# AutonomousVehicleLaboratory/vision_semantic_segmentation

Measured on AMD Instinct MI355X. Metric: fused frames/sec/GPU (1920x1080 + 120k pts) + max|dlog-odds| vs ref, higher is better.
Workload: dtype f16 hi+lo split, MX-FP4 correction passes, fp32 accumulate

## Files before the change

include/avl_hip.h:

```cpp
#ifndef AVL_HIP_H
#define AVL_HIP_H

#include <stdint.h>

#ifdef __cplusplus
extern "C" {
#endif

#define AVL_OK 0
#define AVL_E_ARG (-1)
#define AVL_E_HIP (-2)
#define AVL_E_UNSUPPORTED (-3)

#define AVL_F32 0
#define AVL_F64 1
#define AVL_BF16 2
#define AVL_F16 3

#define AVL_MAX_MAP_CLASSES 16

const char* avl_version(void);
int avl_last_error(char* buf, int len);


// ... 134 lines not shown
    int32_t out_h, out_w, out_c, out_ld, out_rows;
    int32_t in2_ld;
    int32_t ksize, stride, pad, dil, groups;
    int32_t relu;
    int32_t out_f32;
    int32_t w_rows;
    int32_t w_layout;
    int32_t w_split;
    int32_t mx_flags;
    const void* in_lo;
    const void* in2_lo;
    void* out_lo;
    const void* w_mx;
    const void* in_mx;
    void* out_mx;
    const void* in2_mx;
    const void* in3;
    const void* in3_mx;
    int32_t in3_c, in3_ld;
    int32_t batch;
    int32_t bias_per_image;
    int32_t in_format;
    int32_t raw_batch;
} avl_seg_op;

#define AVL_IN_U8_HWC 0
#define AVL_IN_F32_CHW 1

#define AVL_MX_IN_LO 1
#define AVL_MX_RES_LO 2
#define AVL_MX_OUT_LO 4

typedef struct avl_seg_plan avl_seg_plan;

int avl_seg_plan_create(const avl_seg_op* ops_host, int n_ops, avl_seg_plan** out_plan);
void avl_seg_plan_destroy(avl_seg_plan* plan);
int avl_seg_plan_run(avl_seg_plan* plan, void* stream);
int avl_seg_plan_capture(avl_seg_plan* plan, void* stream);
int avl_seg_plan_profile(avl_seg_plan* plan, void* stream, float* ms_host, double* flops_host, double* bytes_host);
int avl_seg_plan_num_ops(const avl_seg_plan* plan);
int avl_seg_plan_nonfinite(avl_seg_plan* plan, void* stream, unsigned long long* counts_host);

#ifdef __cplusplus
}
#endif
#endif
// ... 1 lines not shown
```

vision_semantic_segmentation_amd/csrc/seg_dwpw.hip:

```cpp
#include "seg_types.h"

namespace avl {
namespace {

constexpr int TM = 128;
constexpr int TN = 256;
constexpr int A_STAGE = TM * 128;
constexpr int W_STAGE = TN * 128;
constexpr int LDS_W = 0, LDS_A = 2 * W_STAGE, LDS_P = LDS_A + 2 * A_STAGE;
constexpr int P_STEP = 8 * 6 * 8 * 4;

struct DwPwArgs {
    const void* X;
    const void* X_lo;
    const void* Wc;
    const float* bc;
    float* LG;
    unsigned char* labels;
    int ncls;
    int tiles_x;
    const void* W;
    const float* bias;
    const uint32_t* dwp;
    const int* order;
    int mtiles, per_xcd;
    void* C;
    void* C_lo;
    int H, Wd, OW, ldx, ldc, M, N, K, dil, pad, ntiles;
    unsigned x_bytes;
    int nimg;
};

typedef int v4i __attribute__((ext_vector_type(4)));

__device__ __forceinline__ void dwpw_image(DwPwArgs& p) {
    const long long ipix = (long long)p.H * p.Wd, orows = p.M;
    p.X = image_base(static_cast<const char*>(p.X), ipix, 2LL * p.ldx);
    p.X_lo = image_base(static_cast<const char*>(p.X_lo), ipix, 2LL * p.ldx);
    p.x_bytes -= (unsigned)((long long)blockIdx.z * ipix * p.ldx * 2);
    p.C = image_base(static_cast<char*>(p.C), orows, 2LL * p.ldc);
    p.C_lo = image_base(static_cast<char*>(p.C_lo), orows, 2LL * p.ldc);
    p.LG = image_base(p.LG, orows, p.ncls);
    p.labels = image_base(p.labels, orows, 1);
}

template <typename HT, int WSUB = 1>
__global__ void __launch_bounds__(512) k_dwpw(DwPwArgs p) {
    typedef typename Half16<HT>::v8 v8;
// ... 377 lines not shown
                Vec8<HT>::store(cp + 8, hi);
                if (p.C_lo) {
#pragma unroll
                    for (int i = 0; i < 8; ++i) { lo[i] -= (float)(HT)lo[i]; hi[i] -= (float)(HT)hi[i]; }
                    HT* cl = static_cast<HT*>(p.C_lo) + (long long)m * p.ldc + nbase;
                    Vec8<HT>::store(cl, lo);
                    Vec8<HT>::store(cl + 8, hi);
                }
            }
        }
    }
}

int launch_dwpw_x(const DwPwArgs& a, hipStream_t s) {
    constexpr int lds_bytes = X_LDS_P + XP_RING * FP_STEP;
    static_assert(lds_bytes <= 160 * 1024, "k_dwpw_x LDS");
    AVL_HIP_CHECK(hipFuncSetAttribute(reinterpret_cast<const void*>(&k_dwpw_x), hipFuncAttributeMaxDynamicSharedMemorySize, 160 * 1024));
    hipLaunchKernelGGL(k_dwpw_x, dim3(8 * a.per_xcd * a.ntiles, 1, a.nimg), dim3(512), lds_bytes, s, a);
    AVL_LAUNCH_CHECK();
    return AVL_OK;
}

constexpr int S_LDS_W = 0, S_LDS_AH = 2 * W_STAGE, S_LDS_AL = S_LDS_AH + 2 * A_STAGE, S_LDS_P = S_LDS_AL + 2 * A_STAGE;
template <bool CLS>
__global__ void __launch_bounds__(512) k_dwpw_xs(DwPwArgs p) {
    constexpr int PSTEP = FP_STEP;
    typedef f16 HT;
    typedef typename Half16<HT>::v8 v8;
    extern __shared__ __attribute__((aligned(16))) char lds[];
    const int tid = threadIdx.x, lane = tid & 63;
    const int wave = __builtin_amdgcn_readfirstlane(tid >> 6);
    const int wm = wave >> 2, wn = wave & 3;
    const int nt = blockIdx.x % p.ntiles;
    const int bm = blockIdx.x / p.ntiles, slot = (bm & 7) * p.per_xcd + (bm >> 3);
    if (slot >= p.mtiles) return;
    dwpw_image(p);
    const int mt = p.order[slot];
    const int nk = p.K / 64;

    const unsigned lds0 = lds_addr(lds);
    auto dma_p = [&](int s) {
        if (tid < PSTEP / 16 && s < nk)
            glds16_saddr(reinterpret_cast<const char*>(p.dwp) + s * PSTEP, (unsigned)tid * 16u, lds0 + S_LDS_P + (s & (XP_RING - 1)) * PSTEP + wave * 1024);
    };
    for (int s = 0; s < 3; ++s) dma_p(s);
    const int chunk = tid & 7, r0 = tid >> 3;
    int vbase[2];
    unsigned vmask[2];
    const int tty = p.tiles_x > 0 ? mt / p.tiles_x : 0, ttx = p.tiles_x > 0 ? mt - tty * p.tiles_x : 0;
    const int OHt = p.M / p.OW;
#pragma unroll
    for (int q = 0; q < 2; ++q) {
        const int ml = r0 + q * 64;
        int y, x;
        bool live;
        if (p.tiles_x > 0) {
            y = tty * 8 + (ml >> 4); x = ttx * 16 + (ml & 15);
            live = (y < OHt) & (x < p.OW);
        } else {
            const int m = mt * TM + ml;
            y = m / p.OW; x = m - y * p.OW;
            live = m < p.M;
        }
        vbase[q] = (int)((((long long)(y - p.pad) * p.Wd + (x - p.pad)) * p.ldx + chunk * 8) * 2);
        unsigned mk = 0;
#pragma unroll
        for (int t = 0; t < 9; ++t) {
            const int iy = y - p.pad + (t / 3) * p.dil, ix = x - p.pad + (t % 3) * p.dil;
            mk |= (unsigned)(live & (iy >= 0) & (iy < p.H) & (ix >= 0) & (ix < p.Wd)) << t;
        }
        vmask[q] = mk;
    }
    const int tstep_x = p.dil * p.ldx * 2, tstep_y = p.dil * p.Wd * p.ldx * 2;
    const char* wbase = static_cast<const char*>(p.W) + (long long)nt * TN * p.K * 4;
    unsigned w_voff;
    {
        const int r = wave * 8 + (lane >> 3);
        const int key = ((r >> 1) & 1) | (((r >> 4) & 3) << 1);
        w_voff = (unsigned)(r * p.K * 4 + (((lane & 7) ^ key) << 4));
    }
    const int w_rows64 = 64 * p.K * 4;
    auto dma_w = [&](int h) {
#pragma unroll
        for (int i = 0; i < 4; ++i) glds16_saddr(wbase + h * 128 + i * w_rows64, w_voff, lds0 + S_LDS_W + (h & 1) * W_STAGE + i * 8192 + wave * 1024);
    };
    const int fr = lane & 15, kq = lane >> 4;
    int a_sw[2], w_sw[2];
    {
        const int a_key = fr & 7, w_key = ((fr >> 1) & 1) | (((fr >> 2) & 3) << 1);
#pragma unroll
        for (int kk = 0; kk < 2; ++kk) {
            a_sw[kk] = (wm * 64 + fr) * 128 + (((kk * 4 + kq) ^ a_key) << 4);
            w_sw[kk] = S_LDS_W + (wn * 64 + (fr >> 2) * 16 + (fr & 3)) * 128 + (((kk * 4 + kq) ^ w_key) << 4);
        }
    }
    f32x4 acc[4][4];
    {
        const int nb = nt * TN + wn * 64 + kq * 16;
#pragma unroll
        for (int nj = 0; nj < 4; ++nj) {
            const float4 b = *reinterpret_cast<const float4*>(p.bias + nb + 4 * nj);
#pragma unroll
            for (int mi = 0; mi < 4; ++mi) acc[mi][nj] = f32x4{b.x, b.y, b.z, b.w};
        }
    }

    v4i rh[9], rl[9];
    const __amdgpu_buffer_rsrc_t xrsrc = __builtin_amdgcn_make_buffer_rsrc(const_cast<void*>(p.X), 0, (int)p.x_bytes, 0x00020000);
    const __amdgpu_buffer_rsrc_t xlrsrc = __builtin_amdgcn_make_buffer_rsrc(const_cast<void*>(p.X_lo), 0, (int)p.x_bytes, 0x00020000);
    auto load_taps = [&](int s, int q) {
#pragma unroll
        for (int t = 0; t < 9; ++t) {
            const int off = (vmask[q] >> t) & 1u ? vbase[q] + (t / 3) * tstep_y + (t % 3) * tstep_x : 0x7fffff00;
            rh[t] = __builtin_amdgcn_raw_buffer_load_b128(xrsrc, off, s * 128, 0);
            rl[t] = __builtin_amdgcn_raw_buffer_load_b128(xlrsrc, off, s * 128, 0);
        }
    };

    auto produce_a = [&](int s, int q) {
        float o[8];
        const float* pf = reinterpret_cast<const float*>(lds + S_LDS_P + (s & (XP_RING - 1)) * PSTEP + chunk * (10 * 8 * 4));
        {
            const float4 b0 = *reinterpret_cast<const float4*>(pf + 9 * 8), b1 = *reinterpret_cast<const float4*>(pf + 9 * 8 + 4);
            o[0] = b0.x; o[1] = b0.y; o[2] = b0.z; o[3] = b0.w;
            o[4] = b1.x; o[5] = b1.y; o[6] = b1.z; o[7] = b1.w;
        }
        float wt[9][8];
#pragma unroll
// ... 13 lines not shown
                o[2 * j + 1] = __builtin_fmaf((float)v[1], wt[t][2 * j + 1], o[2 * j + 1]);
            }
#pragma unroll
        for (int t = 0; t < 9; ++t)
#pragma unroll
            for (int j = 0; j < 4; ++j) {
                const int u = rh[t][j];
                const h2 v = __builtin_bit_cast(h2, u);
                o[2 * j] = __builtin_fmaf((float)v[0], wt[t][2 * j], o[2 * j]);
                o[2 * j + 1] = __builtin_fmaf((float)v[1], wt[t][2 * j + 1], o[2 * j + 1]);
            }
        float ol[8];
#pragma unroll
        for (int i = 0; i < 8; ++i) {
            o[i] = fmaxf(o[i], 0.f);
            ol[i] = o[i] - (float)(HT)o[i];
        }
        const int row = r0 + q * 64;
        const int sw = (s & 1) * A_STAGE + row * 128 + ((chunk ^ (row & 7)) << 4);
        Vec8<HT>::store(reinterpret_cast<HT*>(lds + S_LDS_AH + sw), o);
        Vec8<HT>::store(reinterpret_cast<HT*>(lds + S_LDS_AL + sw), ol);
    };

    dma_w(0);
    load_taps(0, 0);
    asm volatile("s_waitcnt vmcnt(18)" ::: "memory");
    __syncthreads();
    produce_a(0, 0);
    load_taps(0, 1);
    produce_a(0, 1);
    if (nk > 1) load_taps(1, 0);

    for (int s = 0; s < nk; ++s) {
        const bool more = s + 1 < nk, more2 = s + 2 < nk;
        const int ts = (s & 1) * A_STAGE;
        auto mfma_hi = [&](int kk) {
            v8 wa[4], ah[4], al[4];
#pragma unroll
            for (int nj = 0; nj < 4; ++nj) wa[nj] = *reinterpret_cast<const v8*>(lds + (kk ? w_sw[1] : w_sw[0]) + nj * 512);
#pragma unroll
            for (int mi = 0; mi < 4; ++mi) {
                ah[mi] = *reinterpret_cast<const v8*>(lds + S_LDS_AH + ts + (kk ? a_sw[1] : a_sw[0]) + mi * 2048);
                al[mi] = *reinterpret_cast<const v8*>(lds + S_LDS_AL + ts + (kk ? a_sw[1] : a_sw[0]) + mi * 2048);
            }
#pragma unroll
            for (int mi = 0; mi < 4; ++mi)
#pragma unroll
                for (int nj = 0; nj < 4; ++nj) acc[mi][nj] = Half16<HT>::mfma(wa[nj], al[mi], acc[mi][nj]);
#pragma unroll
            for (int mi = 0; mi < 4; ++mi)
#pragma unroll
                for (int nj = 0; nj < 4; ++nj) acc[mi][nj] = Half16<HT>::mfma(wa[nj], ah[mi], acc[mi][nj]);
        };
        auto mfma_lo = [&](int kk) {
            v8 wa[4], ah[4];
#pragma unroll
            for (int nj = 0; nj < 4; ++nj) wa[nj] = *reinterpret_cast<const v8*>(lds + W_STAGE + (kk ? w_sw[1] : w_sw[0]) + nj * 512);
#pragma unroll
            for (int mi = 0; mi < 4; ++mi) ah[mi] = *reinterpret_cast<const v8*>(lds + S_LDS_AH + ts + (kk ? a_sw[1] : a_sw[0]) + mi * 2048);
#pragma unroll
            for (int mi = 0; mi < 4; ++mi)
#pragma unroll
                for (int nj = 0; nj < 4; ++nj) acc[mi][nj] = Half16<HT>::mfma(wa[nj], ah[mi], acc[mi][nj]);
        };
        asm volatile("s_waitcnt lgkmcnt(0)" ::: "memory");
        __builtin_amdgcn_s_barrier();
        dma_p(s + 3);
        dma_w(2 * s + 1);
        mfma_hi(0);
        __builtin_amdgcn_sched_barrier(0);
        if (more) { produce_a(s + 1, 0); load_taps(s + 1, 1); }
        __builtin_amdgcn_sched_barrier(0);
        mfma_hi(1);
        if (more) asm volatile("s_waitcnt vmcnt(18)" ::: "memory");
        else asm volatile("s_waitcnt vmcnt(0)" ::: "memory");
        asm volatile("s_waitcnt lgkmcnt(0)" ::: "memory");
        __builtin_amdgcn_s_barrier();
        if (more) dma_w(2 * s + 2);
        mfma_lo(0);
        __builtin_amdgcn_sched_barrier(0);
        if (more) { produce_a(s + 1, 1); if (more2) load_taps(s + 2, 0); }
        __builtin_amdgcn_sched_barrier(0);
        mfma_lo(1);
        if (more2) asm volatile("s_waitcnt vmcnt(18)" ::: "memory");
        else asm volatile("s_waitcnt vmcnt(0)" ::: "memory");
    }

    int elane = lane;
    asm volatile("" : "+v"(elane));
    const int efr = elane & 15;
    if constexpr (CLS) {
        const int ekq = elane >> 4;
        __syncthreads();
#pragma unroll
        for (int mi = 0; mi < 4; ++mi) {
            const int row = wm * 64 + mi * 16 + efr;
            float v0[8], v1[8], l0[8], l1[8];
#pragma unroll
            for (int nj = 0; nj < 2; ++nj)
#pragma unroll
                for (int r = 0; r < 4; ++r) {
                    v0[nj * 4 + r] = fmaxf(acc[mi][nj][r], 0.f);
                    v1[nj * 4 + r] = fmaxf(acc[mi][2 + nj][r], 0.f);
                }
#pragma unroll
            for (int i = 0; i < 8; ++i) { l0[i] = v0[i] - (float)(HT)v0[i]; l1[i] = v1[i] - (float)(HT)v1[i]; }
            const int base = wn * A_STAGE + row * 128;
            const int o0 = base + (((2 * ekq) ^ (row & 7)) << 4), o1 = base + (((2 * ekq + 1) ^ (row & 7)) << 4);
            Vec8<HT>::store(reinterpret_cast<HT*>(lds + o0), v0);
            Vec8<HT>::store(reinterpret_cast<HT*>(lds + o1), v1);
            Vec8<HT>::store(reinterpret_cast<HT*>(lds + 65536 + o0), l0);
            Vec8<HT>::store(reinterpret_cast<HT*>(lds + 65536 + o1), l1);
        }
        __syncthreads();
        f32x4 a2[2];
#pragma unroll
        for (int t2 = 0; t2 < 2; ++t2) {
            const float4 b = *reinterpret_cast<const float4*>(p.bc + t2 * 16 + 4 * ekq);
            a2[t2] = f32x4{b.x, b.y, b.z, b.w};
        }
        const int crow = wave * 16 + efr;
        const char* wcl = static_cast<const char*>(p.Wc) + ((long long)efr * p.N + ekq * 8) * 2;
        const long long wplane = 32LL * p.N * 2;
#pragma unroll
        for (int st = 0; st < 4; ++st)
#pragma unroll
            for (int kk = 0; kk < 2; ++kk) {
                const int off = st * A_STAGE + crow * 128 + (((kk * 4 + ekq) ^ (efr & 7)) << 4);
                const v8 yh = *reinterpret_cast<const v8*>(lds + off), yl = *reinterpret_cast<const v8*>(lds + 65536 + off);
#pragma unroll
                for (int t2 = 0; t2 < 2; ++t2) {
                    const char* wp = wcl + ((long long)t2 * 16 * p.N + st * 64 + kk * 32) * 2;
                    const v8 wh = *reinterpret_cast<const v8*>(wp), wl = *reinterpret_cast<const v8*>(wp + wplane);
                    a2[t2] = Half16<HT>::mfma(wh, yl, a2[t2]);
                    a2[t2] = Half16<HT>::mfma(wl, yh, a2[t2]);
                    a2[t2] = Half16<HT>::mfma(wh, yh, a2[t2]);
                }
            }
        int m;
        {
            const int ml = crow;
            if (p.tiles_x > 0) {
                const int y = tty * 8 + (ml >> 4), x = ttx * 16 + (ml & 15);
                m = ((y < OHt) & (x < p.OW)) ? y * p.OW + x : p.M;
            } else {
                m = mt * TM + ml;
            }
        }
        constexpr int kNone = 1 << 20;
        float best = 0.f;
        int bi = kNone;
#pragma unroll
        for (int t2 = 0; t2 < 2; ++t2)
#pragma unroll
            for (int r = 0; r < 4; ++r) {
                const int cls = t2 * 16 + 4 * ekq + r;
                const float v = a2[t2][r];
                if (cls < p.ncls) {
                    if (m < p.M) p.LG[(long long)m * p.ncls + cls] = v;
                    if (bi == kNone || v > best || (v != v && best == best)) { best = v; bi = cls; }
                }
            }
#pragma unroll
        for (int sh = 16; sh <= 32; sh <<= 1) {
            const float ov = __shfl_xor(best, sh, 64);
            const int oi = __shfl_xor(bi, sh, 64);
            const bool onan = ov != ov, bnan = best != best;
            const bool better = onan ? (!bnan || oi < bi) : (!bnan && (ov > best || (ov == best && oi < bi)));
            if (oi != kNone && (bi == kNone || better)) { best = ov; bi = oi; }
        }
        if (ekq == 0 && m < p.M) p.labels[m] = (unsigned char)bi;
        return;
    }
    const int nbase = nt * TN + wn * 64 + (elane >> 4) * 16;
    if (nbase + 16 <= p.N) {
#pragma unroll
        for (int mi = 0; mi < 4; ++mi) {
            int m = mt * TM + wm * 64 + mi * 16 + efr;
            if (p.tiles_x > 0) {
                const int y = tty * 8 + wm * 4 + mi, x = ttx * 16 + efr;
                m = ((y < OHt) & (x < p.OW)) ? y * p.OW + x : p.M;
            }
            if (m < p.M) {
                float lo[8], hi[8];
#pragma unroll
                for (int nj = 0; nj < 2; ++nj)
#pragma unroll
                    for (int r = 0; r < 4; ++r) {
                        lo[nj * 4 + r] = fmaxf(acc[mi][nj][r], 0.f);
                        hi[nj * 4 + r] = fmaxf(acc[mi][2 + nj][r], 0.f);
                    }
                HT* cp = static_cast<HT*>(p.C) + (long long)m * p.ldc + nbase;
                Vec8<HT>::store(cp, lo);
                Vec8<HT>::store(cp + 8, hi);
                if (p.C_lo) {
#pragma unroll
                    for (int i = 0; i < 8; ++i) { lo[i] -= (float)(HT)lo[i]; hi[i] -= (float)(HT)hi[i]; }
                    HT* cl = static_cast<HT*>(p.C_lo) + (long long)m * p.ldc + nbase;
                    Vec8<HT>::store(cl, lo);
                    Vec8<HT>::store(cl + 8, hi);
                }
            }
        }
    }
}

template <bool CLS>
int launch_dwpw_xs(const DwPwArgs& a, hipStream_t s) {
    constexpr int lds_bytes = S_LDS_P + XP_RING * FP_STEP;
    static_assert(lds_bytes <= 160 * 1024 && S_LDS_AH == 65536 && 4 * A_STAGE == 65536, "k_dwpw_xs LDS (the classifier epilogue keeps y hi at 0 and y lo at 64 KB, 64 KB each)");
    AVL_HIP_CHECK(hipFuncSetAttribute(reinterpret_cast<const void*>(&k_dwpw_xs<CLS>), hipFuncAttributeMaxDynamicSharedMemorySize, 160 * 1024));
    hipLaunchKernelGGL(k_dwpw_xs<CLS>, dim3(8 * a.per_xcd * a.ntiles, 1, a.nimg), dim3(512), lds_bytes, s, a);
    AVL_LAUNCH_CHECK();
    return AVL_OK;
}

template <typename HT, int WSUB>
int launch_dwpw_typed(const DwPwArgs& a, int mtiles, hipStream_t s) {
    const int lds_bytes = LDS_P + (a.K / 64) * P_STEP;
    AVL_HIP_CHECK(hipFuncSetAttribute(reinterpret_cast<const void*>(&k_dwpw<HT, WSUB>), hipFuncAttributeMaxDynamicSharedMemorySize, 160 * 1024));
    hipLaunchKernelGGL((k_dwpw<HT, WSUB>), dim3(8 * a.per_xcd * a.ntiles, 1, a.nimg), dim3(512), lds_bytes, s, a);
    AVL_LAUNCH_CHECK();
    return AVL_OK;
}

}

int validate_dwpw(const avl_seg_op& op) {
    AVL_REQUIRE(is_half(op.dtype), "fused depthwise+pointwise needs a 16-bit activation type");
    AVL_REQUIRE(op.in && op.out && op.weight && op.bias && op.in2, "dwpw has NULL buffers");
    AVL_REQUIRE(!op.w_split || op.dtype == AVL_F16, "split weights need AVL_F16 activations");
    AVL_REQUIRE((!op.in2_lo || op.out_f32) && (!op.out_lo || op.w_split), "dwpw: the output may be split only with w_split (in2_lo: the classifier's bias, with out_f32 only)");
    if (op.out_f32) {
        AVL_REQUIRE(op.w_split == 3 && op.in_lo && !op.out_lo && op.out_c == TN && op.in3 && op.in2_lo && op.out_mx && op.in3_c >= 1 && op.in3_c <= 32 && op.out_ld == op.in3_c,
                    "dwpw with out_f32 (classifier + arg-max in the epilogue): needs a split input, w_split 3, out_c 256, in3 = f16 [2][32][256] weights, in2_lo = "
                    "fp32 bias[32], out = fp32 logits [rows][in3_c <= 32] (out_ld = in3_c), out_mx = uint8 labels[rows], no out_lo");
        AVL_REQUIRE((reinterpret_cast<uintptr_t>(op.in3) | reinterpret_cast<uintptr_t>(op.in2_lo)) % 16 == 0 && reinterpret_cast<uintptr_t>(op.out) % 4 == 0, "dwpw classifier operands unaligned");
    }
    AVL_REQUIRE(op.w_split != 2, "dwpw: w_split 2 (f16 depthwise weight pairs) was replaced by w_split 3 (fp32 depthwise weights)");
    AVL_REQUIRE(!op.in_lo || op.w_split == 3, "dwpw: a split input (in_lo) needs the exact depthwise stage (w_split 3: k_dwpw_xs)");
    AVL_REQUIRE(op.w_layout == 0 || (op.w_layout == 1 && op.in_lo && op.w_split == 3), "dwpw: w_layout 1 (8 x 16-pixel tiles) exists for the split-input kernel only");
    AVL_REQUIRE((reinterpret_cast<uintptr_t>(op.out_lo) | reinterpret_cast<uintptr_t>(op.in_lo)) % 16 == 0, "dwpw low planes must be 16-byte aligned");
    const int M = op.out_h * op.out_w, K = op.in_c, N = op.out_c;
    AVL_REQUIRE(op.stride == 1 && op.ksize == 3 && op.dil >= 1 && op.pad >= 0 && op.out_h == op.in_h + 2 * op.pad - 2 * op.dil &&
                    op.out_w == op.in_w + 2 * op.pad - 2 * op.dil && M > 0,
                "dwpw geometry: 3x3, stride 1, output = input + 2 pad - 2 dilation");
    AVL_REQUIRE(K % 64 == 0 && K <= 2048, "dwpw K = %d (multiple of 64, <= 2048: the depthwise parameters live in LDS)", K);
    AVL_REQUIRE(N % 16 == 0 && op.w_rows >= (N + TN - 1) / TN * TN, "dwpw N = %d / weight rows %d", N, op.w_rows);
    AVL_REQUIRE(op.in_ld >= K && (op.in_ld * 2) % 16 == 0, "dwpw in_ld %d", op.in_ld);
    if (!op.out_f32) AVL_REQUIRE(op.out_ld >= N && (op.out_ld * 2) % 16 == 0, "dwpw out_ld %d", op.out_ld);
    AVL_REQUIRE(op.in_rows >= op.in_h * op.in_w * op_batch(op) && op.out_rows >= M * op_batch(op), "dwpw rows");
    AVL_REQUIRE((long long)op.in_rows * op.in_ld * 2 < 0x7fffff00LL, "dwpw input larger than a buffer descriptor's range");
    AVL_REQUIRE((reinterpret_cast<uintptr_t>(op.in) | reinterpret_cast<uintptr_t>(op.weight) | reinterpret_cast<uintptr_t>(op.out) |
                 reinterpret_cast<uintptr_t>(op.bias) | reinterpret_cast<uintptr_t>(op.in2)) % 16 == 0, "dwpw buffers must be 16-byte aligned");
    return AVL_OK;
}

int launch_dwpw(const avl_seg_op& op, hipStream_t s) {
    DwPwArgs a;
    a.X = op.in; a.X_lo = op.in_lo; a.W = op.weight;
    a.Wc = nullptr; a.bc = nullptr; a.LG = nullptr; a.labels = nullptr; a.ncls = 0;
    a.tiles_x = (op.w_layout == 1) ? (op.out_w + 15) / 16 : 0; a.bias = op.bias; a.dwp = static_cast<const uint32_t*>(op.in2); a.C = op.out;
    a.H = op.in_h; a.Wd = op.in_w; a.OW = op.out_w; a.ldx = op.in_ld; a.ldc = op.out_ld; a.pad = op.pad;
    a.M = op.out_h * op.out_w; a.N = op.out_c; a.K = op.in_c; a.dil = op.dil;
    a.ntiles = (a.N + TN - 1) / TN;
    a.x_bytes = (unsigned)((long long)op.in_rows * op.in_ld * 2);
    a.nimg = op_batch(op);
    const int mtiles = a.tiles_x > 0 ? a.tiles_x * ((op.out_h + 7) / 8) : (a.M + TM - 1) / TM;
    a.mtiles = mtiles;
    a.per_xcd = (mtiles + 7) / 8;
    a.order = reinterpret_cast<const int*>(a.dwp + (a.K / 64) * ((op.w_split == 3 ? FP_STEP : P_STEP) / 4));
    a.C_lo = op.out_lo;
    if (op.w_split == 3 && op.out_f32) {
        a.Wc = op.in3; a.bc = static_cast<const float*>(op.in2_lo); a.LG = static_cast<float*>(op.out); a.labels = static_cast<unsigned char*>(op.out_mx);
        a.ncls = op.in3_c;
        return launch_dwpw_xs<true>(a, s);
    }
    if (op.w_split == 3) return op.in_lo ? launch_dwpw_xs<false>(a, s) : launch_dwpw_x(a, s);
    if (op.w_split) return launch_dwpw_typed<f16, 2>(a, mtiles, s);
    return op.dtype == AVL_F16 ? launch_dwpw_typed<f16, 1>(a, mtiles, s) : launch_dwpw_typed<bf16, 1>(a, mtiles, s);
}

}
```

vision_semantic_segmentation_amd/csrc/seg_plan.hip:

```cpp
#include <vector>

#include "seg_types.h"

struct avl_seg_plan {
    std::vector<avl_seg_op> ops;
    std::vector<hipEvent_t> ev;
    hipGraph_t graph = nullptr;
    hipGraphExec_t exec = nullptr;
};

namespace avl {
namespace {

int validate(const avl_seg_op& op, int index) {
    int rc;
    if (op.batch < 0) rc = set_error(AVL_E_ARG, "batch %d (0 or 1 = one image)", op.batch);
    else if (op.bias_per_image && op.kind != AVL_OP_GEMM) rc = set_error(AVL_E_ARG, "bias_per_image is a GEMM field");
    else if (op.in_format != AVL_IN_U8_HWC && op.in_format != AVL_IN_F32_CHW) rc = set_error(AVL_E_ARG, "in_format %d is not an AVL_IN_* value", op.in_format);
    else if (op.in_format != AVL_IN_U8_HWC && op.kind != AVL_OP_STEM) rc = set_error(AVL_E_ARG, "in_format %d is a stem field (other ops leave it 0)", op.in_format);
    else if (op.in_format == AVL_IN_F32_CHW && op.in2)
        rc = set_error(AVL_E_UNSUPPORTED, op.raw_batch ? "in_format AVL_IN_F32_CHW with raw_batch = 1: a batch of raw frames is uint8 [batch][src_h][src_w][3]"
                                                       : "in_format AVL_IN_F32_CHW with a pre-processing stem (in2 set): that stem reads the raw uint8 frame");
    else if (op.raw_batch != 0 && op.raw_batch != 1) rc = set_error(AVL_E_ARG, "raw_batch %d (0 = one raw frame, 1 = every image of the batch is a raw frame)", op.raw_batch);
    else if (op.raw_batch && op.kind != AVL_OP_STEM) rc = set_error(AVL_E_ARG, "raw_batch is a stem field (other ops leave it 0)");
    else if (op.raw_batch && !op.in2) rc = set_error(AVL_E_ARG, "raw_batch needs a pre-processing stem: in2 (the camera blocks) is NULL");
    else if (op.kind == AVL_OP_GEMM) rc = validate_gemm(op);
    else if (op.kind == AVL_OP_DWPW) rc = validate_dwpw(op);
    else if (op.kind == AVL_OP_BOTTLENECK) rc = validate_bottleneck(op);
    else rc = validate_conv_op(op);
    if (rc != AVL_OK) {
        char msg[400];
        snprintf(msg, sizeof(msg), "%s", err_buf());
        return set_error(rc, "op %d (kind %d): %s", index, op.kind, msg);
    }
    return AVL_OK;
}

int launch(const avl_seg_op& op, hipStream_t s) {
    if (op.kind == AVL_OP_GEMM) return launch_gemm(op, s);
    if (op.kind == AVL_OP_DWPW) return launch_dwpw(op, s);
    if (op.kind == AVL_OP_BOTTLENECK) return launch_bottleneck(op, s);
    return launch_conv_op(op, s);
}

static double act_bytes(double es, bool lo_plane, bool mx, bool mx_lo) {
    double b = es + (lo_plane ? es : 0.0);
    if (mx) b += (mx_lo ? 2.0 : 1.0) * (0.5 + 1.0 / 32.0);
    return b;
// ... 232 lines not shown
```

vision_semantic_segmentation_amd/network.py:

```python
import collections
import ctypes as C
import hashlib
import math

import numpy as np
import torch

from . import _lib

BN_EPS = 1e-5

OP_STEM, OP_MAXPOOL, OP_GEMM, OP_GCONV, OP_DWCONV, OP_BILINEAR, OP_GAP, OP_GEMV, OP_ARGMAX, OP_SUBSAMPLE, OP_DWPW, OP_BOTTLENECK = range(1, 13)
OP_NAMES = {1: "stem", 2: "maxpool", 3: "gemm", 4: "gconv", 5: "dwconv", 6: "bilinear", 7: "gap", 8: "gemv", 9: "argmax", 10: "subsample", 11: "dwpw",
            12: "bottleneck"}


class AvlSegOp(C.Structure):
    _fields_ = [
        ("kind", C.c_int32), ("dtype", C.c_int32),
        ("in_", C.c_void_p), ("in2", C.c_void_p), ("out", C.c_void_p), ("weight", C.c_void_p), ("bias", C.c_void_p),
        ("in_h", C.c_int32), ("in_w", C.c_int32), ("in_c", C.c_int32), ("in_ld", C.c_int32), ("in_rows", C.c_int32),
        ("out_h", C.c_int32), ("out_w", C.c_int32), ("out_c", C.c_int32), ("out_ld", C.c_int32), ("out_rows", C.c_int32),
        ("in2_ld", C.c_int32),
        ("ksize", C.c_int32), ("stride", C.c_int32), ("pad", C.c_int32), ("dil", C.c_int32), ("groups", C.c_int32),
        ("relu", C.c_int32), ("out_f32", C.c_int32), ("w_rows", C.c_int32), ("w_layout", C.c_int32), ("w_split", C.c_int32), ("mx_flags", C.c_int32),
        ("in_lo", C.c_void_p), ("in2_lo", C.c_void_p), ("out_lo", C.c_void_p),
        ("w_mx", C.c_void_p), ("in_mx", C.c_void_p), ("out_mx", C.c_void_p), ("in2_mx", C.c_void_p),
        ("in3", C.c_void_p), ("in3_mx", C.c_void_p), ("in3_c", C.c_int32), ("in3_ld", C.c_int32),
        ("batch", C.c_int32), ("bias_per_image", C.c_int32),
        ("in_format", C.c_int32),
        ("raw_batch", C.c_int32),
    ]


AVL_IN_U8_HWC, AVL_IN_F32_CHW = 0, 1
INPUT_FORMATS = {"u8_hwc": AVL_IN_U8_HWC, "f32_nchw": AVL_IN_F32_CHW}


AVL_MX_IN_LO, AVL_MX_RES_LO, AVL_MX_OUT_LO = 1, 2, 4


_vp, _i = C.c_void_p, C.c_int
_lib._register_seg({
    "avl_seg_plan_create": (_i, [C.POINTER(AvlSegOp), _i, C.POINTER(C.c_void_p)]),
    "avl_seg_plan_destroy": (None, [_vp]),
    "avl_seg_plan_run": (_i, [_vp, _vp]),
    "avl_seg_plan_capture": (_i, [_vp, _vp]),
    "avl_seg_plan_profile": (_i, [_vp, _vp, _vp, _vp, _vp]),
    "avl_seg_plan_num_ops": (_i, [_vp]),
    "avl_seg_plan_nonfinite": (_i, [_vp, _vp, _vp]),
})


PLANES = (64, 128, 256, 512)
# ... 1131 lines not shown
```

Baseline: 228.8.

## Make split-input DWPW kernel persistent with cross-tile prefetch overlap

Turns the k_dwpw_xs kernel into a persistent loop. Each workgroup now walks several M-tiles inside an XCD group, and the grid is sized from the CU count and an optional per-op wg_cap. While the last K step of the current tile runs, it prefetches the next tile's geometry, depthwise weights, pointwise weights and taps, which hides the per-tile prologue. Bias is staged once in LDS, and output stores go through buffer descriptors with an out-of-range offset used to drop masked writes. The cost is more complex synchronisation and register pressure, fewer workgroups to hide latency, and a new struct field that must stay in step between the C and Python sides.

```diff
diff --git a/include/avl_hip.h b/include/avl_hip.h
--- a/include/avl_hip.h
+++ b/include/avl_hip.h
@@ -180,6 +180,7 @@
     int32_t bias_per_image;
     int32_t in_format;
     int32_t raw_batch;
+    int32_t wg_cap;
 } avl_seg_op;
 
 #define AVL_IN_U8_HWC 0
diff --git a/vision_semantic_segmentation_amd/csrc/seg_dwpw.hip b/vision_semantic_segmentation_amd/csrc/seg_dwpw.hip
--- a/vision_semantic_segmentation_amd/csrc/seg_dwpw.hip
+++ b/vision_semantic_segmentation_amd/csrc/seg_dwpw.hip
@@ -24,6 +24,7 @@
     const uint32_t* dwp;
     const int* order;
     int mtiles, per_xcd;
+    int ngrp, per_grp, wpg;
     void* C;
     void* C_lo;
     int H, Wd, OW, ldx, ldc, M, N, K, dil, pad, ntiles;
@@ -447,9 +448,12 @@
 }
 
 constexpr int S_LDS_W = 0, S_LDS_AH = 2 * W_STAGE, S_LDS_AL = S_LDS_AH + 2 * A_STAGE, S_LDS_P = S_LDS_AL + 2 * A_STAGE;
+constexpr int S_LDS_B = S_LDS_P + XP_RING * FP_STEP, S_LDS_BYTES = S_LDS_B + TN * 4;
+typedef unsigned v4u __attribute__((ext_vector_type(4)));
 template <bool CLS>
 __global__ void __launch_bounds__(512) k_dwpw_xs(DwPwArgs p) {
     constexpr int PSTEP = FP_STEP;
+    constexpr unsigned kDrop = 0x80000000u;
     typedef f16 HT;
     typedef typename Half16<HT>::v8 v8;
     extern __shared__ __attribute__((aligned(16))) char lds[];
@@ -457,45 +461,49 @@
     const int wave = __builtin_amdgcn_readfirstlane(tid >> 6);
     const int wm = wave >> 2, wn = wave & 3;
     const int nt = blockIdx.x % p.ntiles;
-    const int bm = blockIdx.x / p.ntiles, slot = (bm & 7) * p.per_xcd + (bm >> 3);
-    if (slot >= p.mtiles) return;
+    const int bm = blockIdx.x / p.ntiles, grp = bm % p.ngrp;
+    const int slot_end = min((grp + 1) * p.per_grp, p.mtiles);
+    int slot = grp * p.per_grp + bm / p.ngrp;
+    if (slot >= slot_end) return;
     dwpw_image(p);
-    const int mt = p.order[slot];
+    int mt = p.order[slot];
     const int nk = p.K / 64;
 
     const unsigned lds0 = lds_addr(lds);
+    if (tid < TN / 4) *reinterpret_cast<float4*>(lds + S_LDS_B + tid * 16) = *reinterpret_cast<const float4*>(p.bias + nt * TN + tid * 4);
     auto dma_p = [&](int s) {
         if (tid < PSTEP / 16 && s < nk)
-            glds16_saddr(reinterpret_cast<const char*>(p.dwp) + s * PSTEP, (unsigned)tid * 16u, lds0 + S_LDS_P + (s & (XP_RING - 1)) * PSTEP + wave * 1024);
-    };
-    for (int s = 0; s < 3; ++s) dma_p(s);
+            glds16_saddr(reinterpret_cast<const char*>(p.dwp) + s * PSTEP, (unsigned)tid * 16u, __builtin_amdgcn_readfirstlane(lds0 + S_LDS_P + (s & (XP_RING - 1)) * PSTEP + wave * 1024));
+    };
     const int chunk = tid & 7, r0 = tid >> 3;
     int vbase[2];
     unsigned vmask[2];
-    const int tty = p.tiles_x > 0 ? mt / p.tiles_x : 0, ttx = p.tiles_x > 0 ? mt - tty * p.tiles_x : 0;
     const int OHt = p.M / p.OW;
-#pragma unroll
-    for (int q = 0; q < 2; ++q) {
-        const int ml = r0 + q * 64;
-        int y, x;
-        bool live;
-        if (p.tiles_x > 0) {
-            y = tty * 8 + (ml >> 4); x = ttx * 16 + (ml & 15);
-            live = (y < OHt) & (x < p.OW);
-        } else {
-            const int m = mt * TM + ml;
-            y = m / p.OW; x = m - y * p.OW;
-            live = m < p.M;
-        }
-        vbase[q] = (int)((((long long)(y - p.pad) * p.Wd + (x - p.pad)) * p.ldx + chunk * 8) * 2);
-        unsigned mk = 0;
-#pragma unroll
-        for (int t = 0; t < 9; ++t) {
-            const int iy = y - p.pad + (t / 3) * p.dil, ix = x - p.pad + (t % 3) * p.dil;
-            mk |= (unsigned)(live & (iy >= 0) & (iy < p.H) & (ix >= 0) & (ix < p.Wd)) << t;
-        }
-        vmask[q] = mk;
-    }
+    auto geometry = [&](int t) {
+        const int tty = p.tiles_x > 0 ? t / p.tiles_x : 0, ttx = p.tiles_x > 0 ? t - tty * p.tiles_x : 0;
+#pragma unroll
+        for (int q = 0; q < 2; ++q) {
+            const int ml = r0 + q * 64;
+            int y, x;
+            bool live;
+            if (p.tiles_x > 0) {
+                y = tty * 8 + (ml >> 4); x = ttx * 16 + (ml & 15);
+                live = (y < OHt) & (x < p.OW);
+            } else {
+                const int m = t * TM + ml;
+                y = m / p.OW; x = m - y * p.OW;
+                live = m < p.M;
+            }
+            vbase[q] = (int)((((long long)(y - p.pad) * p.Wd + (x - p.pad)) * p.ldx + chunk * 8) * 2);
+            unsigned mk = 0;
+#pragma unroll
+            for (int tp = 0; tp < 9; ++tp) {
+                const int iy = y - p.pad + (tp / 3) * p.dil, ix = x - p.pad + (tp % 3) * p.dil;
+                mk |= (unsigned)(live & (iy >= 0) & (iy < p.H) & (ix >= 0) & (ix < p.Wd)) << tp;
+            }
+            vmask[q] = mk;
+        }
+    };
     const int tstep_x = p.dil * p.ldx * 2, tstep_y = p.dil * p.Wd * p.ldx * 2;
     const char* wbase = static_cast<const char*>(p.W) + (long long)nt * TN * p.K * 4;
     unsigned w_voff;
@@ -507,7 +515,7 @@
     const int w_rows64 = 64 * p.K * 4;
     auto dma_w = [&](int h) {
 #pragma unroll
-        for (int i = 0; i < 4; ++i) glds16_saddr(wbase + h * 128 + i * w_rows64, w_voff, lds0 + S_LDS_W + (h & 1) * W_STAGE + i * 8192 + wave * 1024);
+        for (int i = 0; i < 4; ++i) glds16_saddr(wbase + h * 128 + i * w_rows64, w_voff, __builtin_amdgcn_readfirstlane(lds0 + S_LDS_W + (h & 1) * W_STAGE + i * 8192 + wave * 1024));
     };
     const int fr = lane & 15, kq = lane >> 4;
     int a_sw[2], w_sw[2];
@@ -520,15 +528,6 @@
         }
     }
     f32x4 acc[4][4];
-    {
-        const int nb = nt * TN + wn * 64 + kq * 16;
-#pragma unroll
-        for (int nj = 0; nj < 4; ++nj) {
-            const float4 b = *reinterpret_cast<const float4*>(p.bias + nb + 4 * nj);
-#pragma unroll
-            for (int mi = 0; mi < 4; ++mi) acc[mi][nj] = f32x4{b.x, b.y, b.z, b.w};
-        }
-    }
 
     v4i rh[9], rl[9];
     const __amdgpu_buffer_rsrc_t xrsrc = __builtin_amdgcn_make_buffer_rsrc(const_cast<void*>(p.X), 0, (int)p.x_bytes, 0x00020000);
@@ -588,166 +587,215 @@
         Vec8<HT>::store(reinterpret_cast<HT*>(lds + S_LDS_AL + sw), ol);
     };
 
+    auto store8 = [&](const __amdgpu_buffer_rsrc_t& r, unsigned off, const float (&v)[8]) {
+        f16x8 x;
+#pragma unroll
+        for (int i = 0; i < 8; ++i) x[i] = (f16)v[i];
+        __builtin_amdgcn_raw_buffer_store_b128(__builtin_bit_cast(v4u, x), r, (int)off, 0, 0);
+    };
+
+    geometry(mt);
+    for (int s = 0; s < 3; ++s) dma_p(s);
     dma_w(0);
     load_taps(0, 0);
     asm volatile("s_waitcnt vmcnt(18)" ::: "memory");
-    __syncthreads();
-    produce_a(0, 0);
-    load_taps(0, 1);
-    produce_a(0, 1);
-    if (nk > 1) load_taps(1, 0);
-
-    for (int s = 0; s < nk; ++s) {
-        const bool more = s + 1 < nk, more2 = s + 2 < nk;
-        const int ts = (s & 1) * A_STAGE;
-        auto mfma_hi = [&](int kk) {
-            v8 wa[4], ah[4], al[4];
-#pragma unroll
-            for (int nj = 0; nj < 4; ++nj) wa[nj] = *reinterpret_cast<const v8*>(lds + (kk ? w_sw[1] : w_sw[0]) + nj * 512);
-#pragma unroll
-            for (int mi = 0; mi < 4; ++mi) {
-                ah[mi] = *reinterpret_cast<const v8*>(lds + S_LDS_AH + ts + (kk ? a_sw[1] : a_sw[0]) + mi * 2048);
-                al[mi] = *reinterpret_cast<const v8*>(lds + S_LDS_AL + ts + (kk ? a_sw[1] : a_sw[0]) + mi * 2048);
-            }
-#pragma unroll
-            for (int mi = 0; mi < 4; ++mi)
-#pragma unroll
-                for (int nj = 0; nj < 4; ++nj) acc[mi][nj] = Half16<HT>::mfma(wa[nj], al[mi], acc[mi][nj]);
-#pragma unroll
-            for (int mi = 0; mi < 4; ++mi)
-#pragma unroll
-                for (int nj = 0; nj < 4; ++nj) acc[mi][nj] = Half16<HT>::mfma(wa[nj], ah[mi], acc[mi][nj]);
-        };
-        auto mfma_lo = [&](int kk) {
-            v8 wa[4], ah[4];
-#pragma unroll
-            for (int nj = 0; nj < 4; ++nj) wa[nj] = *reinterpret_cast<const v8*>(lds + W_STAGE + (kk ? w_sw[1] : w_sw[0]) + nj * 512);
-#pragma unroll
-            for (int mi = 0; mi < 4; ++mi) ah[mi] = *reinterpret_cast<const v8*>(lds + S_LDS_AH + ts + (kk ? a_sw[1] : a_sw[0]) + mi * 2048);
-#pragma unroll
-            for (int mi = 0; mi < 4; ++mi)
-#pragma unroll
-                for (int nj = 0; nj < 4; ++nj) acc[mi][nj] = Half16<HT>::mfma(wa[nj], ah[mi], acc[mi][nj]);
-        };
+
+    for (;;) {
+        const int nslot = slot + p.wpg;
+        const bool has_next = nslot < slot_end;
+        int mt_next = 0;
+        if (has_next) asm volatile("s_load_dword %0, %1, 0x0\n\ts_waitcnt lgkmcnt(0)" : "=s"(mt_next) : "s"(p.order + nslot) : "memory");
         asm volatile("s_waitcnt lgkmcnt(0)" ::: "memory");
         __builtin_amdgcn_s_barrier();
-        dma_p(s + 3);
-        dma_w(2 * s + 1);
-        mfma_hi(0);
-        __builtin_amdgcn_sched_barrier(0);
-        if (more) { produce_a(s + 1, 0); load_taps(s + 1, 1); }
-        __builtin_amdgcn_sched_barrier(0);
-        mfma_hi(1);
-        if (more) asm volatile("s_waitcnt vmcnt(18)" ::: "memory");
-        else asm volatile("s_waitcnt vmcnt(0)" ::: "memory");
-        asm volatile("s_waitcnt lgkmcnt(0)" ::: "memory");
-        __builtin_amdgcn_s_barrier();
-        if (more) dma_w(2 * s + 2);
-        mfma_lo(0);
-        __builtin_amdgcn_sched_barrier(0);
-        if (more) { produce_a(s + 1, 1); if (more2) load_taps(s + 2, 0); }
-        __builtin_amdgcn_sched_barrier(0);
-        mfma_lo(1);
-        if (more2) asm volatile("s_waitcnt vmcnt(18)" ::: "memory");
-        else asm volatile("s_waitcnt vmcnt(0)" ::: "memory");
-    }
-
-    int elane = lane;
-    asm volatile("" : "+v"(elane));
-    const int efr = elane & 15;
-    if constexpr (CLS) {
-        const int ekq = elane >> 4;
-        __syncthreads();
-#pragma unroll
-        for (int mi = 0; mi < 4; ++mi) {
-            const int row = wm * 64 + mi * 16 + efr;
-            float v0[8], v1[8], l0[8], l1[8];
-#pragma unroll
-            for (int nj = 0; nj < 2; ++nj)
+        asm volatile("" ::: "memory");
+        {
+            const float* bl = reinterpret_cast<const float*>(lds + S_LDS_B) + wn * 64 + kq * 16;
+#pragma unroll
+            for (int nj = 0; nj < 4; ++nj) {
+                const float4 b = *reinterpret_cast<const float4*>(bl + 4 * nj);
+#pragma unroll
+                for (int mi = 0; mi < 4; ++mi) acc[mi][nj] = f32x4{b.x, b.y, b.z, b.w};
+            }
+        }
+        produce_a(0, 0);
+        load_taps(0, 1);
+        produce_a(0, 1);
+        if (nk > 1) load_taps(1, 0);
+
+        for (int s = 0; s < nk; ++s) {
+            const bool more = s + 1 < nk, more2 = s + 2 < nk;
+            const int ts = (s & 1) * A_STAGE;
+            auto mfma_hi = [&](int kk) {
+                v8 wa[4], ah[4], al[4];
+#pragma unroll
+                for (int nj = 0; nj < 4; ++nj) wa[nj] = *reinterpret_cast<const v8*>(lds + (kk ? w_sw[1] : w_sw[0]) + nj * 512);
+#pragma unroll
+                for (int mi = 0; mi < 4; ++mi) {
+                    ah[mi] = *reinterpret_cast<const v8*>(lds + S_LDS_AH + ts + (kk ? a_sw[1] : a_sw[0]) + mi * 2048);
+                    al[mi] = *reinterpret_cast<const v8*>(lds + S_LDS_AL + ts + (kk ? a_sw[1] : a_sw[0]) + mi * 2048);
+                }
+#pragma unroll
+                for (int mi = 0; mi < 4; ++mi)
+#pragma unroll
+                    for (int nj = 0; nj < 4; ++nj) acc[mi][nj] = Half16<HT>::mfma(wa[nj], al[mi], acc[mi][nj]);
+#pragma unroll
+                for (int mi = 0; mi < 4; ++mi)
+#pragma unroll
+                    for (int nj = 0; nj < 4; ++nj) acc[mi][nj] = Half16<HT>::mfma(wa[nj], ah[mi], acc[mi][nj]);
+            };
+            auto mfma_lo = [&](int kk) {
+                v8 wa[4], ah[4];
+#pragma unroll
+                for (int nj = 0; nj < 4; ++nj) wa[nj] = *reinterpret_cast<const v8*>(lds + W_STAGE + (kk ? w_sw[1] : w_sw[0]) + nj * 512);
+#pragma unroll
+                for (int mi = 0; mi < 4; ++mi) ah[mi] = *reinterpret_cast<const v8*>(lds + S_LDS_AH + ts + (kk ? a_sw[1] : a_sw[0]) + mi * 2048);
+#pragma unroll
+                for (int mi = 0; mi < 4; ++mi)
+#pragma unroll
+                    for (int nj = 0; nj < 4; ++nj) acc[mi][nj] = Half16<HT>::mfma(wa[nj], ah[mi], acc[mi][nj]);
+            };
+            asm volatile("s_waitcnt lgkmcnt(0)" ::: "memory");
+            __builtin_amdgcn_s_barrier();
+            dma_p(s + 3);
+            dma_w(2 * s + 1);
+            mfma_hi(0);
+            __builtin_amdgcn_sched_barrier(0);
+            if (more) { produce_a(s + 1, 0); load_taps(s + 1, 1); }
+            __builtin_amdgcn_sched_barrier(0);
+            mfma_hi(1);
+            if (more) asm volatile("s_waitcnt vmcnt(18)" ::: "memory");
+            else asm volatile("s_waitcnt vmcnt(0)" ::: "memory");
+            asm volatile("s_waitcnt lgkmcnt(0)" ::: "memory");
+            __builtin_amdgcn_s_barrier();
+            if (more) dma_w(2 * s + 2);
+            mfma_lo(0);
+            __builtin_amdgcn_sched_barrier(0);
+            if (more) {
+                produce_a(s + 1, 1);
+                if (more2) load_taps(s + 2, 0);
+            } else if (has_next) {
+                geometry(mt_next);
+                for (int s2 = 0; s2 < 3; ++s2) dma_p(s2);
+                if constexpr (!CLS) dma_w(0);
+                load_taps(0, 0);
+            }
+            __builtin_amdgcn_sched_barrier(0);
+            mfma_lo(1);
+            if (more2) asm volatile("s_waitcnt vmcnt(18)" ::: "memory");
+            else if (more || !has_next) asm volatile("s_waitcnt vmcnt(0)" ::: "memory");
+        }
+
+        int elane = lane;
+        asm volatile("" : "+v"(elane));
+        const int efr = elane & 15;
+        const int tty = p.tiles_x > 0 ? mt / p.tiles_x : 0, ttx = p.tiles_x > 0 ? mt - tty * p.tiles_x : 0;
+        if constexpr (CLS) {
+            const int ekq = elane >> 4;
+            asm volatile("s_waitcnt lgkmcnt(0)" ::: "memory");
+            __builtin_amdgcn_s_barrier();
+            asm volatile("" ::: "memory");
+#pragma unroll
+            for (int mi = 0; mi < 4; ++mi) {
+                const int row = wm * 64 + mi * 16 + efr;
+                float v0[8], v1[8], l0[8], l1[8];
+#pragma unroll
+                for (int nj = 0; nj < 2; ++nj)
+#pragma unroll
+                    for (int r = 0; r < 4; ++r) {
+                        v0[nj * 4 + r] = fmaxf(acc[mi][nj][r], 0.f);
+                        v1[nj * 4 + r] = fmaxf(acc[mi][2 + nj][r], 0.f);
+                    }
+#pragma unroll
+                for (int i = 0; i < 8; ++i) { l0[i] = v0[i] - (float)(HT)v0[i]; l1[i] = v1[i] - (float)(HT)v1[i]; }
+                const int base = wn * A_STAGE + row * 128;
+                const int o0 = base + (((2 * ekq) ^ (row & 7)) << 4), o1 = base + (((2 * ekq + 1) ^ (row & 7)) << 4);
+                Vec8<HT>::store(reinterpret_cast<HT*>(lds + o0), v0);
+                Vec8<HT>::store(reinterpret_cast<HT*>(lds + o1), v1);
+                Vec8<HT>::store(reinterpret_cast<HT*>(lds + 65536 + o0), l0);
+                Vec8<HT>::store(reinterpret_cast<HT*>(lds + 65536 + o1), l1);
+            }
+            asm volatile("s_waitcnt lgkmcnt(0)" ::: "memory");
+            __builtin_amdgcn_s_barrier();
+            asm volatile("" ::: "memory");
+            f32x4 a2[2];
+#pragma unroll
+            for (int t2 = 0; t2 < 2; ++t2) {
+                const float4 b = *reinterpret_cast<const float4*>(p.bc + t2 * 16 + 4 * ekq);
+                a2[t2] = f32x4{b.x, b.y, b.z, b.w};
+            }
+            const int crow = wave * 16 + efr;
+            const char* wcl = static_cast<const char*>(p.Wc) + ((long long)efr * p.N + ekq * 8) * 2;
+            const long long wplane = 32LL * p.N * 2;
+#pragma unroll
+            for (int st = 0; st < 4; ++st)
+#pragma unroll
+                for (int kk = 0; kk < 2; ++kk) {
+                    const int off = st * A_STAGE + crow * 128 + (((kk * 4 + ekq) ^ (efr & 7)) << 4);
+                    const v8 yh = *reinterpret_cast<const v8*>(lds + off), yl = *reinterpret_cast<const v8*>(lds + 65536 + off);
+#pragma unroll
+                    for (int t2 = 0; t2 < 2; ++t2) {
+                        const char* wp = wcl + ((long long)t2 * 16 * p.N + st * 64 + kk * 32) * 2;
+                        const v8 wh = *reinterpret_cast<const v8*>(wp), wl = *reinterpret_cast<const v8*>(wp + wplane);
+                        a2[t2] = Half16<HT>::mfma(wh, yl, a2[t2]);
+                        a2[t2] = Half16<HT>::mfma(wl, yh, a2[t2]);
+                        a2[t2] = Half16<HT>::mfma(wh, yh, a2[t2]);
+                    }
+                }
+            if (has_next) {
+                asm volatile("s_waitcnt lgkmcnt(0)" ::: "memory");
+                __builtin_amdgcn_s_barrier();
+                dma_w(0);
+            }
+            int m;
+            {
+                const int ml = crow;
+                if (p.tiles_x > 0) {
+                    const int y = tty * 8 + (ml >> 4), x = ttx * 16 + (ml & 15);
+                    m = ((y < OHt) & (x < p.OW)) ? y * p.OW + x : p.M;
+                } else {
+                    m = mt * TM + ml;
+                }
+            }
+            const __amdgpu_buffer_rsrc_t lgrsrc = __builtin_amdgcn_make_buffer_rsrc(p.LG, 0, p.M * p.ncls * 4, 0x00020000);
+            const __amdgpu_buffer_rsrc_t lbrsrc = __builtin_amdgcn_make_buffer_rsrc(p.labels, 0, p.M, 0x00020000);
+            constexpr int kNone = 1 << 20;
+            float best = 0.f;
+            int bi = kNone;
+#pragma unroll
+            for (int t2 = 0; t2 < 2; ++t2)
 #pragma unroll
                 for (int r = 0; r < 4; ++r) {
-                    v0[nj * 4 + r] = fmaxf(acc[mi][nj][r], 0.f);
-                    v1[nj * 4 + r] = fmaxf(acc[mi][2 + nj][r], 0.f);
+                    const int cls = t2 * 16 + 4 * ekq + r;
+                    const float v = a2[t2][r];
+                    const bool real = cls < p.ncls;
+                    __builtin_amdgcn_raw_buffer_store_b32(__float_as_uint(v), lgrsrc, (int)((real & (m < p.M)) ? (unsigned)(m * p.ncls + cls) * 4u : kDrop), 0, 0);
+                    if (real && (bi == kNone || v > best || (v != v && best == best))) { best = v; bi = cls; }
                 }
 #pragma unroll
-            for (int i = 0; i < 8; ++i) { l0[i] = v0[i] - (float)(HT)v0[i]; l1[i] = v1[i] - (float)(HT)v1[i]; }
-            const int base = wn * A_STAGE + row * 128;
-            const int o0 = base + (((2 * ekq) ^ (row & 7)) << 4), o1 = base + (((2 * ekq + 1) ^ (row & 7)) << 4);
-            Vec8<HT>::store(reinterpret_cast<HT*>(lds + o0), v0);
-            Vec8<HT>::store(reinterpret_cast<HT*>(lds + o1), v1);
-            Vec8<HT>::store(reinterpret_cast<HT*>(lds + 65536 + o0), l0);
-            Vec8<HT>::store(reinterpret_cast<HT*>(lds + 65536 + o1), l1);
-        }
-        __syncthreads();
-        f32x4 a2[2];
-#pragma unroll
-        for (int t2 = 0; t2 < 2; ++t2) {
-            const float4 b = *reinterpret_cast<const float4*>(p.bc + t2 * 16 + 4 * ekq);
-            a2[t2] = f32x4{b.x, b.y, b.z, b.w};
-        }
-        const int crow = wave * 16 + efr;
-        const char* wcl = static_cast<const char*>(p.Wc) + ((long long)efr * p.N + ekq * 8) * 2;
-        const long long wplane = 32LL * p.N * 2;
-#pragma unroll
-        for (int st = 0; st < 4; ++st)
-#pragma unroll
-            for (int kk = 0; kk < 2; ++kk) {
-                const int off = st * A_STAGE + crow * 128 + (((kk * 4 + ekq) ^ (efr & 7)) << 4);
-                const v8 yh = *reinterpret_cast<const v8*>(lds + off), yl = *reinterpret_cast<const v8*>(lds + 65536 + off);
-#pragma unroll
-                for (int t2 = 0; t2 < 2; ++t2) {
-                    const char* wp = wcl + ((long long)t2 * 16 * p.N + st * 64 + kk * 32) * 2;
-                    const v8 wh = *reinterpret_cast<const v8*>(wp), wl = *reinterpret_cast<const v8*>(wp + wplane);
-                    a2[t2] = Half16<HT>::mfma(wh, yl, a2[t2]);
-                    a2[t2] = Half16<HT>::mfma(wl, yh, a2[t2]);
-                    a2[t2] = Half16<HT>::mfma(wh, yh, a2[t2]);
+            for (int sh = 16; sh <= 32; sh <<= 1) {
+                const float ov = __shfl_xor(best, sh, 64);
+                const int oi = __shfl_xor(bi, sh, 64);
+                const bool onan = ov != ov, bnan = best != best;
+                const bool better = onan ? (!bnan || oi < bi) : (!bnan && (ov > best || (ov == best && oi < bi)));
+                if (oi != kNone && (bi == kNone || better)) { best = ov; bi = oi; }
+            }
+            __builtin_amdgcn_raw_buffer_store_b8((unsigned char)bi, lbrsrc, (int)(((ekq == 0) & (m < p.M)) ? (unsigned)m : kDrop), 0, 0);
+            if (!has_next) break;
+            asm volatile("s_waitcnt vmcnt(9)" ::: "memory");
+        } else {
+            const int nbase = nt * TN + wn * 64 + (elane >> 4) * 16;
+            const bool cols = nbase + 16 <= p.N;
+            const int out_bytes = p.M * p.ldc * 2;
+            const __amdgpu_buffer_rsrc_t orsrc = __builtin_amdgcn_make_buffer_rsrc(p.C, 0, out_bytes, 0x00020000);
+            const __amdgpu_buffer_rsrc_t olrsrc = __builtin_amdgcn_make_buffer_rsrc(p.C_lo ? p.C_lo : p.C, 0, out_bytes, 0x00020000);
+#pragma unroll
+            for (int mi = 0; mi < 4; ++mi) {
+                int m = mt * TM + wm * 64 + mi * 16 + efr;
+                if (p.tiles_x > 0) {
+                    const int y = tty * 8 + wm * 4 + mi, x = ttx * 16 + efr;
+                    m = ((y < OHt) & (x < p.OW)) ? y * p.OW + x : p.M;
                 }
-            }
-        int m;
-        {
-            const int ml = crow;
-            if (p.tiles_x > 0) {
-                const int y = tty * 8 + (ml >> 4), x = ttx * 16 + (ml & 15);
-                m = ((y < OHt) & (x < p.OW)) ? y * p.OW + x : p.M;
-            } else {
-                m = mt * TM + ml;
-            }
-        }
-        constexpr int kNone = 1 << 20;
-        float best = 0.f;
-        int bi = kNone;
-#pragma unroll
-        for (int t2 = 0; t2 < 2; ++t2)
-#pragma unroll
-            for (int r = 0; r < 4; ++r) {
-                const int cls = t2 * 16 + 4 * ekq + r;
-                const float v = a2[t2][r];
-                if (cls < p.ncls) {
-                    if (m < p.M) p.LG[(long long)m * p.ncls + cls] = v;
-                    if (bi == kNone || v > best || (v != v && best == best)) { best = v; bi = cls; }
-                }
-            }
-#pragma unroll
-        for (int sh = 16; sh <= 32; sh <<= 1) {
-            const float ov = __shfl_xor(best, sh, 64);
-            const int oi = __shfl_xor(bi, sh, 64);
-            const bool onan = ov != ov, bnan = best != best;
-            const bool better = onan ? (!bnan || oi < bi) : (!bnan && (ov > best || (ov == best && oi < bi)));
-            if (oi != kNone && (bi == kNone || better)) { best = ov; bi = oi; }
-        }
-        if (ekq == 0 && m < p.M) p.labels[m] = (unsigned char)bi;
-        return;
-    }
-    const int nbase = nt * TN + wn * 64 + (elane >> 4) * 16;
-    if (nbase + 16 <= p.N) {
-#pragma unroll
-        for (int mi = 0; mi < 4; ++mi) {
-            int m = mt * TM + wm * 64 + mi * 16 + efr;
-            if (p.tiles_x > 0) {
-                const int y = tty * 8 + wm * 4 + mi, x = ttx * 16 + efr;
-                m = ((y < OHt) & (x < p.OW)) ? y * p.OW + x : p.M;
-            }
-            if (m < p.M) {
+                const unsigned ooff = (cols & (m < p.M)) ? (unsigned)(m * p.ldc + nbase) * 2u : kDrop;
                 float lo[8], hi[8];
 #pragma unroll
                 for (int nj = 0; nj < 2; ++nj)
@@ -756,27 +804,45 @@
                         lo[nj * 4 + r] = fmaxf(acc[mi][nj][r], 0.f);
                         hi[nj * 4 + r] = fmaxf(acc[mi][2 + nj][r], 0.f);
                     }
-                HT* cp = static_cast<HT*>(p.C) + (long long)m * p.ldc + nbase;
-                Vec8<HT>::store(cp, lo);
-                Vec8<HT>::store(cp + 8, hi);
+                store8(orsrc, ooff, lo);
+                store8(orsrc, ooff + 16u, hi);
                 if (p.C_lo) {
 #pragma unroll
                     for (int i = 0; i < 8; ++i) { lo[i] -= (float)(HT)lo[i]; hi[i] -= (float)(HT)hi[i]; }
-                    HT* cl = static_cast<HT*>(p.C_lo) + (long long)m * p.ldc + nbase;
-                    Vec8<HT>::store(cl, lo);
-                    Vec8<HT>::store(cl + 8, hi);
+                    store8(olrsrc, ooff, lo);
+                    store8(olrsrc, ooff + 16u, hi);
                 }
             }
-        }
-    }
+            if (!has_next) break;
+            if (p.C_lo) asm volatile("s_waitcnt vmcnt(16)" ::: "memory");
+            else asm volatile("s_waitcnt vmcnt(8)" ::: "memory");
+        }
+        slot = nslot;
+        mt = mt_next;
+    }
+}
+
+static int device_cus() {
+    static int n = 0;
+    if (n == 0) {
+        int dev = 0;
+        hipDeviceProp_t prop;
+        if (hipGetDevice(&dev) == hipSuccess && hipGetDeviceProperties(&prop, dev) == hipSuccess) n = prop.multiProcessorCount;
+        if (n <= 0) n = 256;
+    }
+    return n;
 }
 
 template <bool CLS>
-int launch_dwpw_xs(const DwPwArgs& a, hipStream_t s) {
-    constexpr int lds_bytes = S_LDS_P + XP_RING * FP_STEP;
-    static_assert(lds_bytes <= 160 * 1024 && S_LDS_AH == 65536 && 4 * A_STAGE == 65536, "k_dwpw_xs LDS (the classifier epilogue keeps y hi at 0 and y lo at 64 KB, 64 KB each)");
+int launch_dwpw_xs(DwPwArgs a, int wg_cap, hipStream_t s) {
+    static_assert(S_LDS_BYTES <= 160 * 1024 && S_LDS_AH == 65536 && 4 * A_STAGE == 65536, "k_dwpw_xs LDS (the classifier epilogue keeps y hi at 0 and y lo at 64 KB, 64 KB each)");
+    const int per_cu = device_cus() / a.ntiles > 0 ? device_cus() / a.ntiles : 1;
+    const int wgs = wg_cap > 0 && wg_cap < per_cu ? wg_cap : per_cu;
+    a.ngrp = wgs < 8 ? wgs : 8;
+    a.per_grp = (a.mtiles + a.ngrp - 1) / a.ngrp;
+    a.wpg = wgs / a.ngrp < a.per_grp ? wgs / a.ngrp : a.per_grp;
     AVL_HIP_CHECK(hipFuncSetAttribute(reinterpret_cast<const void*>(&k_dwpw_xs<CLS>), hipFuncAttributeMaxDynamicSharedMemorySize, 160 * 1024));
-    hipLaunchKernelGGL(k_dwpw_xs<CLS>, dim3(8 * a.per_xcd * a.ntiles, 1, a.nimg), dim3(512), lds_bytes, s, a);
+    hipLaunchKernelGGL(k_dwpw_xs<CLS>, dim3(a.ngrp * a.wpg * a.ntiles, 1, a.nimg), dim3(512), S_LDS_BYTES, s, a);
     AVL_LAUNCH_CHECK();
     return AVL_OK;
 }
@@ -805,6 +871,7 @@
     }
     AVL_REQUIRE(op.w_split != 2, "dwpw: w_split 2 (f16 depthwise weight pairs) was replaced by w_split 3 (fp32 depthwise weights)");
     AVL_REQUIRE(!op.in_lo || op.w_split == 3, "dwpw: a split input (in_lo) needs the exact depthwise stage (w_split 3: k_dwpw_xs)");
+    AVL_REQUIRE(op.wg_cap >= 0 && (!op.wg_cap || (op.in_lo && op.w_split == 3)), "dwpw: wg_cap %d (>= 0; it bounds the persistent split-input kernel's workgroups, other forms leave it 0)", op.wg_cap);
     AVL_REQUIRE(op.w_layout == 0 || (op.w_layout == 1 && op.in_lo && op.w_split == 3), "dwpw: w_layout 1 (8 x 16-pixel tiles) exists for the split-input kernel only");
     AVL_REQUIRE((reinterpret_cast<uintptr_t>(op.out_lo) | reinterpret_cast<uintptr_t>(op.in_lo)) % 16 == 0, "dwpw low planes must be 16-byte aligned");
     const int M = op.out_h * op.out_w, K = op.in_c, N = op.out_c;
@@ -817,6 +884,7 @@
     if (!op.out_f32) AVL_REQUIRE(op.out_ld >= N && (op.out_ld * 2) % 16 == 0, "dwpw out_ld %d", op.out_ld);
     AVL_REQUIRE(op.in_rows >= op.in_h * op.in_w * op_batch(op) && op.out_rows >= M * op_batch(op), "dwpw rows");
     AVL_REQUIRE((long long)op.in_rows * op.in_ld * 2 < 0x7fffff00LL, "dwpw input larger than a buffer descriptor's range");
+    if (op.in_lo) AVL_REQUIRE((long long)M * op.out_ld * (op.out_f32 ? 4 : 2) < 0x7fffff00LL, "dwpw: one image's output is larger than a buffer descriptor's range");
     AVL_REQUIRE((reinterpret_cast<uintptr_t>(op.in) | reinterpret_cast<uintptr_t>(op.weight) | reinterpret_cast<uintptr_t>(op.out) |
                  reinterpret_cast<uintptr_t>(op.bias) | reinterpret_cast<uintptr_t>(op.in2)) % 16 == 0, "dwpw buffers must be 16-byte aligned");
     return AVL_OK;
@@ -835,14 +903,15 @@
     const int mtiles = a.tiles_x > 0 ? a.tiles_x * ((op.out_h + 7) / 8) : (a.M + TM - 1) / TM;
     a.mtiles = mtiles;
     a.per_xcd = (mtiles + 7) / 8;
+    a.ngrp = 8; a.per_grp = a.per_xcd; a.wpg = a.per_xcd;
     a.order = reinterpret_cast<const int*>(a.dwp + (a.K / 64) * ((op.w_split == 3 ? FP_STEP : P_STEP) / 4));
     a.C_lo = op.out_lo;
     if (op.w_split == 3 && op.out_f32) {
         a.Wc = op.in3; a.bc = static_cast<const float*>(op.in2_lo); a.LG = static_cast<float*>(op.out); a.labels = static_cast<unsigned char*>(op.out_mx);
         a.ncls = op.in3_c;
-        return launch_dwpw_xs<true>(a, s);
-    }
-    if (op.w_split == 3) return op.in_lo ? launch_dwpw_xs<false>(a, s) : launch_dwpw_x(a, s);
+        return launch_dwpw_xs<true>(a, op.wg_cap, s);
+    }
+    if (op.w_split == 3) return op.in_lo ? launch_dwpw_xs<false>(a, op.wg_cap, s) : launch_dwpw_x(a, s);
     if (op.w_split) return launch_dwpw_typed<f16, 2>(a, mtiles, s);
     return op.dtype == AVL_F16 ? launch_dwpw_typed<f16, 1>(a, mtiles, s) : launch_dwpw_typed<bf16, 1>(a, mtiles, s);
 }
diff --git a/vision_semantic_segmentation_amd/csrc/seg_plan.hip b/vision_semantic_segmentation_amd/csrc/seg_plan.hip
--- a/vision_semantic_segmentation_amd/csrc/seg_plan.hip
+++ b/vision_semantic_segmentation_amd/csrc/seg_plan.hip
@@ -24,6 +24,7 @@
     else if (op.raw_batch != 0 && op.raw_batch != 1) rc = set_error(AVL_E_ARG, "raw_batch %d (0 = one raw frame, 1 = every image of the batch is a raw frame)", op.raw_batch);
     else if (op.raw_batch && op.kind != AVL_OP_STEM) rc = set_error(AVL_E_ARG, "raw_batch is a stem field (other ops leave it 0)");
     else if (op.raw_batch && !op.in2) rc = set_error(AVL_E_ARG, "raw_batch needs a pre-processing stem: in2 (the camera blocks) is NULL");
+    else if (op.wg_cap && op.kind != AVL_OP_DWPW) rc = set_error(AVL_E_ARG, "wg_cap is a DWPW field (other ops leave it 0)");
     else if (op.kind == AVL_OP_GEMM) rc = validate_gemm(op);
     else if (op.kind == AVL_OP_DWPW) rc = validate_dwpw(op);
     else if (op.kind == AVL_OP_BOTTLENECK) rc = validate_bottleneck(op);
diff --git a/vision_semantic_segmentation_amd/network.py b/vision_semantic_segmentation_amd/network.py
--- a/vision_semantic_segmentation_amd/network.py
+++ b/vision_semantic_segmentation_amd/network.py
@@ -30,6 +30,7 @@
         ("batch", C.c_int32), ("bias_per_image", C.c_int32),
         ("in_format", C.c_int32),
         ("raw_batch", C.c_int32),
+        ("wg_cap", C.c_int32),
     ]
 
 
```

After: 225.7. -1.4%, worse.
